# adam-kerrigan/pybader

Hardware: AMD Instinct MI355X
Metric: Mvoxels/s neargrid assign+refine on 512^3 grid (higher is better)
Workload: dtype f64; 1 GPU; 512^3 synthetic 8-Gaussian-atom cubic cell (BASELINE config 3), neargrid assign + neargrid edge refinement changed:2, density resident in HBM; method=neargrid, device_driven_slab_step=False, basins=8

## Files before the change

include/bader_hip.h:

```cpp
#ifndef BADER_HIP_H
#define BADER_HIP_H

#include <stdint.h>

#ifdef __cplusplus
extern "C" {
#endif

typedef struct xb_ctx xb_ctx;

enum { XB_OK = 0, XB_E_ARG = -1, XB_E_HIP = -2, XB_E_STATE = -3, XB_E_LIMIT = -4, XB_E_COMM = -5,
       XB_E_SHORT = -6  };

enum { XB_I8 = 1, XB_I16 = 2, XB_I32 = 4, XB_I64 = 8 };

enum { XB_METHOD_ONGRID = 0, XB_METHOD_NEARGRID = 1 };
enum { XB_REFINE_ALL = 0, XB_REFINE_CHANGED = 1 };

const char *xb_last_error(void);
int xb_device_count(void);
int xb_create(int device, xb_ctx **out);
void xb_destroy(xb_ctx *c);
int xb_sync(xb_ctx *c);
void *xb_stream(xb_ctx *c);
// ... 228 lines not shown
    XB_REGIONS_BOXES = 1,
    XB_REGIONS_BRICKS = 2
};
enum { XB_DROP_TABLE_AND_MAXIMA = 2 };
enum {
    XB_CHECK_NO_MIRROR = 1,
    XB_CHECK_GENERIC_WALKER = 2,
    XB_CHECK_FULL_TGRAD = 4,
    XB_CHECK_LIST_DILATE = 8,
    XB_CHECK_WIDE_HALO = 16,
    XB_CHECK_NO_EC_SHARE = 32,
    XB_CHECK_IO_GATHER = 64
};
#define XB_CHECK_BRICK_LOOKUP 128
#define XB_CHECK_VOXEL_SWEEP 256
#define XB_CHECK_GENERIC_RETRACE 512
enum {
    XB_DBG_EC_PASSES = 4,
    XB_DBG_SLAB_STATS = 16,
    XB_DBG_STAGE_WAIT = 32,
    XB_DBG_SHORT_TIERS = 64
};
#define XB_DBG_KEEP_RETRACE_OVERFLOW 128
int xb_set_option(xb_ctx *c, int key, int value);
int xb_host_alloc(int64_t bytes, void **out);
int xb_host_free(void *p);
int xb_memory_stats(xb_ctx *c, int64_t *bytes_total, int64_t *bytes_table, int64_t *bytes_scratch);
int xb_box_stats(xb_ctx *c, int64_t *n_boxes, int64_t *box_voxels);
int xb_brick_labels(xb_ctx *c, int32_t *out, int64_t capacity, int64_t dims[3]);
int xb_slow_path_stats(xb_ctx *c, int64_t *assign_total, int64_t *refine_total);
int xb_deferred_stats(xb_ctx *c, int64_t *refine_total);
int xb_sweep_stats(xb_ctx *c, int64_t *bit_sweeps, int64_t *voxel_sweeps);
int xb_retrace_stats(xb_ctx *c, int64_t *lean_launches, int64_t *generic_launches);
int xb_retrace_overflow(xb_ctx *c, int32_t *out, int64_t capacity, int64_t *n);
int xb_edge_list(xb_ctx *c, int32_t *out, int64_t capacity, int64_t *edges, int64_t *tiles_listed);
int xb_growth_stats(xb_ctx *c, int64_t *retries, int64_t *kill_launches);

int xb_comm_unique_id(uint8_t id_out[128]);
int xb_comm_init(xb_ctx *c, int rank, int nranks, const uint8_t id_in[128]);
int xb_comm_destroy(xb_ctx *c);
int xb_comm_exchange_planes(xb_ctx *c, int which, int n_send, const int32_t *send_peer, const int64_t *send_xa,
                            const int64_t *send_xb, int n_recv, const int32_t *recv_peer, const int64_t *recv_xa,
                            const int64_t *recv_xb);
int xb_comm_allreduce_i64(xb_ctx *c, int64_t *inout, int64_t n, int op);
int xb_comm_allgather_i64(xb_ctx *c, const int64_t *in, int64_t n, int64_t *out);
int xb_comm_share_brick_masks(xb_ctx *c, const int64_t *first, const int64_t *count);
int xb_comm_allgather_block(xb_ctx *c, int which, const int64_t *first, const int64_t *count);
int xb_comm_allreduce_block(xb_ctx *c);
int xb_comm_info(xb_ctx *c, int64_t out[4]);
int xb_comm_stats(xb_ctx *c, int64_t *bytes_sent);

#ifdef __cplusplus
}
#endif
#endif
```

pybader_amd/_lib.py:

```python
import ctypes as C
import threading
import os

import numpy as np

HERE = os.path.dirname(os.path.abspath(__file__))
LIB_PATH = os.environ.get('XB_LIBRARY') or os.path.join(HERE, 'libbader_hip.so')

METHODS = {'ongrid': 0, 'neargrid': 1}
REFINE_MODES = {'all': 0, 'changed': 1}
DTYPE_CODE = {np.dtype(np.int8): 1, np.dtype(np.int16): 2, np.dtype(np.int32): 4, np.dtype(np.int64): 8}
(XB_XC_EDGES, XB_XC_CHANGED, XB_XC_ESCAPED, XB_XC_TRAVELLING, XB_XC_SLOW, XB_XC_LOST, XB_XC_MINE, XB_XC_ROUNDS,
 XB_XC_COUNT) = range(9)
(XB_TIMER_ASSIGN, XB_TIMER_OG_MASKS, XB_TIMER_EDGE_FIND, XB_TIMER_REFINE_TRACE, XB_TIMER_MASKS_GROWTH, XB_TIMER_BRICK_MASKS,
 XB_TIMER_TRACE, XB_TIMER_BRICK_RECORDS, XB_TIMER_MOMENTS, XB_TIMER_ADJACENCY, XB_TIMER_MERGE, XB_TIMER_COUNT) = range(12)
XB_OPT_REGIONS = 1
XB_REGIONS_BOXES, XB_REGIONS_BRICKS = 1, 2
XB_OPT_CROSS_CHECK = 2
(XB_CHECK_NO_MIRROR, XB_CHECK_GENERIC_WALKER, XB_CHECK_FULL_TGRAD, XB_CHECK_LIST_DILATE, XB_CHECK_WIDE_HALO,
 XB_CHECK_NO_EC_SHARE, XB_CHECK_IO_GATHER) = (1, 2, 4, 8, 16, 32, 64)
CROSS_CHECK_BRICK_LOOKUP = 128
CROSS_CHECK_VOXEL_SWEEP = 256
CROSS_CHECK_GENERIC_RETRACE = 512
XB_OPT_DEBUG = 3
# ... 147 lines not shown
    'xb_isa_rho_bound': (_int, [_vp, _pdbl]),
    'xb_volume_assign': (_int, [_vp, _vp, _i64]),
    'xb_atom_assign': (_int, [_vp, _i64, _vp, _i64, _vp, _vp, _vp]),
    'xb_surface_distance': (_int, [_vp, _vp, _vp, _i64, _vp, _pi64]),
    'xb_volume_mask': (_int, [_vp, _i64, _vp]),
    'xb_label_sum': (_int, [_vp, _i64, _pdbl, _pi64]),
    'xb_set_table_window': (_int, [_vp, _i64]),
    'xb_table_build': (_int, [_vp, _pi64]),
    'xb_table_local_seeds': (_int, [_vp, _vp, _i64]),
    'xb_brick_masks': (_int, [_vp, C.POINTER(_vp), _pi64, _pi64, _pi64]),
    'xb_table_ties': (_int, [_vp, _pi64]),
    'xb_table_finish': (_int, [_vp, _vp, _i64, _i64]),
    'xb_labels_ptr': (_vp, [_vp]),
    'xb_known_ptr': (_vp, [_vp]),
    'xb_density_ptr': (_vp, [_vp]),
    'xb_plane_elems': (_i64, [_vp]),
    'xb_copy_planes': (_int, [_vp, _int, _int, _vp, _i64, _i64]),
    'xb_label_wire': (_int, [_vp, _int, _vp]),
    'xb_host_alloc': (_int, [_i64, _vp]),
    'xb_host_free': (_int, [_vp]),
    'xb_brick_masks_copy': (_int, [_vp, _int, _vp, _i64, _i64]),
    'xb_set_halo': (_int, [_vp, _i64]),
    'xb_kernel_time': (_int, [_vp, _int, _pdbl, _pi64]),
    'xb_kernel_time_reset': (_int, [_vp]),
    'xb_enable_timing': (_int, [_vp, _int]),
    'xb_set_option': (_int, [_vp, _int, _int]),
    'xb_box_stats': (_int, [_vp, _pi64, _pi64]),
    'xb_brick_labels': (_int, [_vp, _vp, _i64, _pi64]),
    'xb_slow_path_stats': (_int, [_vp, _pi64, _pi64]),
    'xb_deferred_stats': (_int, [_vp, _pi64]),
    'xb_sweep_stats': (_int, [_vp, _pi64, _pi64]),
    'xb_edge_list': (_int, [_vp, _vp, _i64, _pi64, _pi64]),
    'xb_retrace_stats': (_int, [_vp, _pi64, _pi64]),
    'xb_retrace_overflow': (_int, [_vp, _vp, _i64, _pi64]),
    'xb_growth_stats': (_int, [_vp, _pi64, _pi64]),
    'xb_comm_unique_id': (_int, [_vp]),
    'xb_comm_init': (_int, [_vp, _int, _int, _vp]),
    'xb_comm_destroy': (_int, [_vp]),
    'xb_comm_exchange_planes': (_int, [_vp, _int, _int, _vp, _pi64, _pi64, _int, _vp, _pi64, _pi64]),
    'xb_comm_allreduce_i64': (_int, [_vp, _pi64, C.c_int64, _int]),
    'xb_comm_allgather_i64': (_int, [_vp, _pi64, C.c_int64, _pi64]),
    'xb_comm_share_brick_masks': (_int, [_vp, _pi64, _pi64]),
    'xb_comm_allgather_block': (_int, [_vp, _int, _pi64, _pi64]),
    'xb_comm_allreduce_block': (_int, [_vp]),
    'xb_slab_supported': (_int, [_vp, _int, _pi64]),
    'xb_slab_assign_masks': (_int, [_vp, _int, _int]),
    'xb_slab_assign_trace': (_int, [_vp]),
    'xb_slab_assign_finish': (_int, [_vp, _pi64, _pi64]),
    'xb_slab_refine_pass': (_int, [_vp]),
    'xb_slab_walkers_round': (_int, [_vp, _int, _int]),
    'xb_slab_walk_layout': (_int, [_vp, _pi64]),
    'xb_slab_walk_send': (_int, [_vp, _i64]),
    'xb_slab_refine_counts': (_int, [_vp, _pi64, _pi64]),
    'xb_slab_block': (_int, [_vp, _int, C.POINTER(_vp), _pi64, _pi64, _pi64]),
    'xb_slab_block_copy': (_int, [_vp, _int, _int, _vp, _i64, _i64]),
    'xb_host_waits': (_int, [_pi64]),
    'xb_comm_stats': (_int, [_vp, _pi64]),
    'xb_comm_info': (_int, [_vp, _pi64]),
    'xb_memory_stats': (_int, [_vp, _pi64, _pi64, _pi64]),
}

_lib = None


class BaderHipError(RuntimeError):
    code = None
# ... 1045 lines not shown

    def brick_labels(self):
        dims = (C.c_int64 * 3)()
        check(self.lib.xb_brick_labels(self.h, None, 0, dims))
        out = np.zeros(tuple(int(d) for d in dims), np.int32)
        check(self.lib.xb_brick_labels(self.h, _ptr(out), out.size, dims))
        return out

    def slow_path_stats(self):
        a, b = C.c_int64(), C.c_int64()
        check(self.lib.xb_slow_path_stats(self.h, C.byref(a), C.byref(b)))
        return a.value, b.value

    def growth_stats(self):
        a, b = C.c_int64(), C.c_int64()
        check(self.lib.xb_growth_stats(self.h, C.byref(a), C.byref(b)))
        return a.value, b.value

    def deferred_stats(self):
        a = C.c_int64()
        check(self.lib.xb_deferred_stats(self.h, C.byref(a)))
        return a.value

    def sweep_stats(self):
        a, b = C.c_int64(), C.c_int64()
        check(self.lib.xb_sweep_stats(self.h, C.byref(a), C.byref(b)))
        return a.value, b.value

    def retrace_stats(self):
        a, b = C.c_int64(), C.c_int64()
        check(self.lib.xb_retrace_stats(self.h, C.byref(a), C.byref(b)))
        return a.value, b.value

    def retrace_overflow(self):
        n = C.c_int64()
        check(self.lib.xb_retrace_overflow(self.h, None, 0, C.byref(n)))
        out = np.zeros(n.value, np.int32)
        if n.value:
            check(self.lib.xb_retrace_overflow(self.h, _ptr(out), out.size, C.byref(n)))
        return out

    def edge_list(self):
        n, t = C.c_int64(), C.c_int64()
        check(self.lib.xb_edge_list(self.h, None, 0, C.byref(n), C.byref(t)))
        out = np.zeros(n.value, np.int32)
        if n.value:
            check(self.lib.xb_edge_list(self.h, _ptr(out), out.size, C.byref(n), C.byref(t)))
        return out, t.value

    def sync(self):
        check(self.lib.xb_sync(self.h))


def critical_lut():
    out = np.zeros(XB_CRITICAL_LUT_SIZE, np.uint8)
    check(load().xb_critical_lut(_ptr(out)))
    return out


def isosurface_table():
    out = np.zeros(XB_ISO_TABLE_SIZE, np.uint8)
    check(load().xb_isosurface_table(_ptr(out)))
    return out.reshape(6, 16, 8)


def hirshfeld_images(lattice, atoms_cart, species, r_cut):
# ... 40 lines not shown
```

pybader_amd/csrc/bader_hip.hip:

```cpp
#include "bader_kernels.h"
#include "../../include/bader_hip.h"
#include "ctx_state.h"
#include "ctx_buffers.h"

#include <algorithm>
#include <cmath>
#include <cstdarg>
#include <cstdio>
#include <cstring>
#include <locale.h>
#include <mutex>
#include <string>
#include <thread>
#include <vector>

static thread_local long long xb_waits = 0;
static inline hipError_t xb_counted_sync(hipStream_t s) { xb_waits++; return (hipStreamSynchronize)(s); }
#define hipStreamSynchronize(s) xb_counted_sync(s)

#include "k_common.h"
#include "k_masks.h"
#include "k_fused.h"
#include "k_trace.h"
#include "k_ongrid.h"
// ... 77 lines not shown
        int ec_qcap = EC_Q;
        int self_exchange = 0;
        int async_comm = 0;
        bool weight_no_labels = false;
    } opt;
    int *ec_share = nullptr;
    std::vector<int64_t> esc_starts, esc_offsets, esc_vox;
    unsigned long long *ec_pend = nullptr;
    int8_t *ec_pflag = nullptr;
    std::vector<int8_t> esc_complete;
    double vac_tol = 0.;
    bool regions_pending = false;
    bool buni_halo_safe = false;
    bool regions_neargrid = false;
    int n_walk = 0;
    int *walk = nullptr;
    int table_margin = -1;
    bool table_prebuilt = false;
    int table_stage = 0;
    std::vector<int> window_seeds;
    bool window_ties = true;
    bool slab_sparse = false;
    int ec_local_n = 0;
    int walk_n_out = 0;
    void *walk_out_dev = nullptr;
    std::vector<int64_t> walk_host, res_host;
    int walk_n_res = 0;
    void *walk_in = nullptr, *walk_out2 = nullptr, *walk_res = nullptr;
    long long walk_cap = 0;
    long long stat_deferred = 0;
    long long stat_bit_sweeps = 0, stat_voxel_sweeps = 0;
    long long stat_ovf_assign = 0, stat_ovf_refine = 0;
    long long stat_lean_retraces = 0, stat_generic_retraces = 0;
    std::vector<int> dbg_retrace_ovf;
    int *bres_last = nullptr;
    int *blab = nullptr;
    int nbk[3] = {0, 0, 0};
    bool brick_max_blanket = false;
    int grad_cover = 0;
    unsigned char *brick_rec = nullptr;
    unsigned long long *nb_tab = nullptr;
    void *xbuf = nullptr;
    int slab_rank = 0, slab_nranks = 0, slab_stage = 0;
    void *wbuf[2] = {nullptr, nullptr};
    void *wk_in = nullptr;
    int wbuf_ranks = 0, walk_last = -1, walk_round = 0, wcap = 0;
    int walk_send = 0;
    int grow_kill_launches = 6;
    long long stat_grow_retries = 0;
    bool defer_wait = false;
    bool pending_assign = false;
    int64_t pending_n_maxima = 0;
    int grad_rule = 0;
    int *labels = nullptr;
    int8_t *known = nullptr;
    int *first = nullptr;
    int *list = nullptr;
    int8_t *st = nullptr;
    void *stage = nullptr;
    size_t stage_bytes = 0;
    int *max_list = nullptr;
    int *max_aux = nullptr;
    int max_cap = 0;
    int *ovf_list = nullptr;
    int ovf_cap = 0;
    int *counters = nullptr;
// ... 204 lines not shown
    case XB_OPT_DROP_TABLE: if (value == XB_DROP_TABLE_AND_MAXIMA) drop_table_and_maxima(*c); else drop_table(*c); break;
    case XB_OPT_KILL_LAUNCHES: if ((ok = value >= 1)) c->grow_kill_launches = value; break;
    case XB_OPT_SELF_EXCHANGE: c->opt.self_exchange = value != 0; break;
    case XB_OPT_ASYNC_COMM: c->opt.async_comm = value != 0; break;
    case XB_OPT_WEIGHT_NO_LABELS: c->opt.weight_no_labels = value != 0; break;
    default: ok = false;
    }
    if (!ok) return fail(XB_E_ARG, "xb_set_option: unknown key %d", key);
    return XB_OK;
}
int xb_growth_stats(xb_ctx *c, int64_t *retries, int64_t *kill_launches) {
    if (!c) return fail(XB_E_ARG, "null ctx");
    if (retries) *retries = c->stat_grow_retries;
    if (kill_launches) *kill_launches = c->grow_kill_launches;
    return XB_OK;
}
int xb_deferred_stats(xb_ctx *c, int64_t *refine_total) {
    if (!c) return fail(XB_E_ARG, "null ctx");
    if (refine_total) *refine_total = c->stat_deferred;
    return XB_OK;
}
int xb_sweep_stats(xb_ctx *c, int64_t *bit_sweeps, int64_t *voxel_sweeps) {
    if (!c) return fail(XB_E_ARG, "null ctx");
    if (bit_sweeps) *bit_sweeps = c->stat_bit_sweeps;
    if (voxel_sweeps) *voxel_sweeps = c->stat_voxel_sweeps;
    return XB_OK;
}
int xb_retrace_stats(xb_ctx *c, int64_t *lean_launches, int64_t *generic_launches) {
    if (!c) return fail(XB_E_ARG, "null ctx");
    if (lean_launches) *lean_launches = c->stat_lean_retraces;
    if (generic_launches) *generic_launches = c->stat_generic_retraces;
    return XB_OK;
}
int xb_retrace_overflow(xb_ctx *c, int32_t *out, int64_t capacity, int64_t *n) {
    if (!c || !n || capacity < 0 || (capacity > 0 && !out)) return fail(XB_E_ARG, "xb_retrace_overflow: null ctx / count, or a capacity without a buffer");
    *n = (int64_t)c->dbg_retrace_ovf.size();
    if (capacity >= *n) {
        std::copy(c->dbg_retrace_ovf.begin(), c->dbg_retrace_ovf.end(), out);
        c->dbg_retrace_ovf.clear();
    }
    return XB_OK;
}
int xb_slow_path_stats(xb_ctx *c, int64_t *assign_total, int64_t *refine_total) {
    if (!c) return fail(XB_E_ARG, "null ctx");
    if (assign_total) *assign_total = c->stat_ovf_assign;
    if (refine_total) *refine_total = c->stat_ovf_refine;
    return XB_OK;
}
int xb_memory_stats(xb_ctx *c, int64_t *bytes_total, int64_t *bytes_table, int64_t *bytes_scratch) {
    if (!c || !c->has_grid) return fail(XB_E_STATE, "xb_memory_stats: no grid");
    const long long N = c->N;
    const long long table = c->grad_cap * (long long)sizeof(GradRec);
    const long long scratch = c->list_cap * 4 + (long long)c->stage_bytes + c->ec_buf_cap * 4 + (c->ec_pend ? 8 * N + 16 : 0) +
                              (long long)buf_counted_bytes(*c) ;
    const long long fixed = 8 * N  + 4 * N  + (N + 16)  + 4 * N  + N  +
                            2LL * c->max_cap * 4 + (long long)c->ovf_cap * 4 + c->blab_alloc * 13 + (long long)c->walk_cap * 3 * 80 +
                            (1 << 22) ;
    if (bytes_total) *bytes_total = fixed + table + scratch;
    if (bytes_table) *bytes_table = table;
    if (bytes_scratch) *bytes_scratch = scratch;
    return XB_OK;
}
int xb_box_stats(xb_ctx *c, int64_t *n_boxes, int64_t *box_voxels) {
    if (!c) return fail(XB_E_ARG, "null ctx");
    if (n_boxes) *n_boxes = c->n_boxes;
    if (box_voxels) *box_voxels = c->box_voxels;
// ... 76 lines not shown
```

pybader_amd/csrc/bader_kernels.h:

```cpp
#pragma once
#include <hip/hip_runtime.h>
#include <stdint.h>

struct Grid {
    int nx, ny, nz;
    int nyz;
    int x0, x1;
    int vx0, vlen;
    int wx0, wlen;
    int wbase, ntot;
    int main_ties;
    double T[9];
    double dist[27];
};

struct GridS {
    int nx, ny, nz, nyz;
    int x0, x1, vx0, vlen;
    int wx0, wlen;
    int wbase, ntot;
    int main_ties;
    double T[9];
    double dsym[14];
};
// ... 113 lines not shown
#define XB_KEY_BITS 21
#define XB_NB_SHIFT 11
constexpr __host__ __device__ int nb_side(int pos) { return pos < 4 ? -1 : 1; }
constexpr __host__ __device__ int nb_index(int cx, int cy, int cz) { return cx + 2 * cy + 4 * cz - 1; }
constexpr __host__ __device__ int key_low(int code, int og, int nb) { return code | (og << 6) | ((nb & 127) << XB_NB_SHIFT); }
constexpr __host__ __device__ int low_code(int bits) { return bits & 63; }
constexpr __host__ __device__ int low_og(int bits) { return (bits >> 6) & 31; }
constexpr __host__ __device__ bool low_nb_norec(int bits, int cx, int cy, int cz) {
    return (cx | cy | cz) != 0 && ((bits >> (XB_NB_SHIFT + nb_index(cx, cy, cz))) & 1) != 0;
}
namespace nb_check {
constexpr bool subsets_ok() {
    for (int m = 1; m < 8; m++) {
        const int cx = m & 1, cy = (m >> 1) & 1, cz = m >> 2;
        if (nb_index(cx, cy, cz) != m - 1) return false;
        for (int code = 0; code < 64; code += 21)
            for (int og = 0; og < 27; og += 13) {
                const int one = key_low(code, og, 1 << (m - 1)), rest = key_low(code, og, 127 & ~(1 << (m - 1)));
                if (low_code(one) != code || low_og(one) != og || low_code(rest) != code || low_og(rest) != og) return false;
                if (one >> XB_KEY_BITS || rest >> XB_KEY_BITS) return false;
                for (int k = 1; k < 8; k++) {
                    if (low_nb_norec(one, k & 1, (k >> 1) & 1, k >> 2) != (k == m)) return false;
                    if (low_nb_norec(rest, k & 1, (k >> 1) & 1, k >> 2) != (k != m)) return false;
                }
                if (low_nb_norec(one, 0, 0, 0) || low_nb_norec(key_low(code, og, 127), 0, 0, 0)) return false;
            }
    }
    return true;
}
static_assert(subsets_ok(), "7 neighbour bits, one per subset of crossed axes, clear of the step code and the ongrid successor");
static_assert(nb_side(0) == -1 && nb_side(1) == -1 && nb_side(3) == -1 && nb_side(4) == 1 && nb_side(6) == 1 && nb_side(7) == 1,
              "the low side is within reach from positions 0-1 only, the high side from 6-7 only");
static_assert(key_low(XB_STAY_CODE, 26, 127) == 0x3FEBF && key_low(63, 31, 127) < (1 << 18), "bits 18-20 stay 0");
}
__device__ __forceinline__ double pack_key(double rho, int code, int og, int nb = 0) {
    return __longlong_as_double((__double_as_longlong(rho) & ~0x1FFFFFLL) | (long long)key_low(code, og, nb));
}
__device__ __forceinline__ double key_floor(double rho) {
    const long long b = __double_as_longlong(rho);
    return __longlong_as_double(b >= 0 ? (b & ~0x1FFFFFLL) : (b | 0x1FFFFFLL));
}
__device__ __forceinline__ int key_bits(double key) { return (int)(__double_as_longlong(key) & 0x1FFFFFLL); }
__device__ __forceinline__ int key_code(double key) { return low_code(key_bits(key)); }
__device__ __forceinline__ int key_og(double key) { return low_og(key_bits(key)); }
static_assert((1 << XB_KEY_BITS) - 1 == 0x1FFFFF, "key_bits / key_floor / pack_key share one mask");

__device__ __forceinline__ int wrap_u(int q, int n) {
    unsigned u = min((unsigned)q, (unsigned)(q + n));
    return (int)min(u, u - (unsigned)n);
}
__device__ __forceinline__ int lin3f(const GridL &g, int x, int y, int z) {
    if (g.use24) return (int)__umul24(__umul24(x, g.ny) + y, g.nz) + z;
    return (x * g.ny + y) * g.nz + z;
}
__device__ __forceinline__ void ng_move_t(const GridL &g, int px, int py, int pz, const GradRec &rec, int code,
                                          double &dr0, double &dr1, double &dr2, int &qx, int &qy, int &qz) {
    int id;
    dr0 += rec.r0; id = rha_cs(dr0); qx = px + ((code & 3) - 1) + id; dr0 -= (double)id;
    dr1 += rec.r1; id = rha_cs(dr1); qy = py + (((code >> 2) & 3) - 1) + id; dr1 -= (double)id;
    dr2 += rec.r2; id = rha_cs(dr2); qz = pz + ((code >> 4) - 1) + id; dr2 -= (double)id;
    qx = wrap_u(qx, g.nx); qy = wrap_u(qy, g.ny); qz = wrap_u(qz, g.nz);
}

template <typename GT>
__device__ __forceinline__ void og_step(const double *__restrict__ rho, const GT &g, const double *__restrict__ dist,
                                        int px, int py, int pz, double ctr, int &qx, int &qy, int &qz) {
// ... 89 lines not shown
```

pybader_amd/csrc/host_stages.h:

```cpp

enum { BB_TOTAL = 1 << 20, BB_REGMAX = 1 << 16, BB_REGFIRST = 1 << 17 };

static bool table_windowed(const xb_ctx *c) { return c->g.wlen < c->g.nx; }
static int small_grid(const Grid &g) { return g.nx < 16 || g.ny < 16 || g.nz < 80; }
static int trace_maxsteps(const Grid &g) { return 8 * (g.nx + g.ny + g.nz) + 64; }
static const int *slab_regions_of(const xb_ctx *c) {
    const Grid &g = c->g;
    return (table_windowed(c) && c->blab && c->regions_labels && !c->has_vacuum && (c->grad_rule == 2 || c->slab_sparse) &&
            g.nx % 8 == 0 && g.ny % 8 == 0 && g.nz % 8 == 0) ? c->blab : nullptr;
}

static_assert(CT_REDO == CT_N_MAX + 15, "a host-driven assignment zeroes CT_N_MAX .. CT_REDO at once");
static int begin_assignment(xb_ctx *c, int *counts, int n, bool invalidate) {
    HIPCHK(hipMemsetAsync(counts, 0, n * sizeof(int), c->stream));
    if (!c->first_clean) {
        k_fill<int><<<4096, TPB, 0, c->stream>>>(c->first, XB_INT_MAX, c->N);
        HIPCHK(hipGetLastError());
    }
    c->first_clean = false;
    c->regions_pending = false;
    if (invalidate) { drop_label_marks(*c); drop_edge_lists(*c); }
    return XB_OK;
}

// ... 37 lines not shown
    const int nbr = nb0 * nb1 * nb2;
    int *fs = c->fs;
    k_seed_bricks<<<(nbr + 255) / 256, 256, 0, c->stream>>>(nbr, bmask, bmaxv, fs, seed, buf0, box_max, box_first);
    if (chase) {
        k_grow_parent<<<(nbr + TPB - 1) / TPB, TPB, 0, c->stream>>>(nb0, nb1, nb2, bmask, bpot, seed, buf1);
        k_grow_chase<<<(nbr + TPB - 1) / TPB, TPB, 0, c->stream>>>(nbr, buf1, seed, buf0, 4 * (nb0 + nb1 + nb2) + 64, fs);
    } else
        k_seed_finish<<<1, 1, 0, c->stream>>>(fs);
    const int long_schedule = 2 * ((std::max(std::max(nb0, nb1), nb2) + BG - 1) / BG) + 12;
    const int launches = chase ? std::min(long_schedule, c->grow_kill_launches) : long_schedule;
    const dim3 ggrid((nb2 + BG - 1) / BG, (nb1 + BG - 1) / BG, (nb0 + BG - 1) / BG);
    for (int l = 0; l < launches; l++)
        k_brick_grow_dev<<<ggrid, BG * BG * BG, 0, c->stream>>>(nb0, nb1, nb2, bmask, seed, buf0, buf1, fs, BG, 0);
    k_grow_finish<<<64, TPB, 0, c->stream>>>(nbr, seed, buf0, buf1, fs, c->blab_buf, box_first, bmask, c->brick_rec, 0, chase && launches < long_schedule ? 1 : 0);
}

static void launch_window_bricks(xb_ctx *c, int *list, int *count, const int *skip) {
    const Grid &g = c->g;
    const int nb0 = c->nbk[0], per_plane = c->nbk[1] * c->nbk[2], nbr = nb0 * per_plane;
    const int w0 = g.wx0 / BRK, wn = g.wlen / BRK, run1 = std::min(wn, nb0 - w0);
    const unsigned grid = (nbr + 16 * TPB - 1) / (16 * TPB);
    k_brick_walk_list<<<grid, TPB, 0, c->stream>>>(nbr, w0 * per_plane, (w0 + run1) * per_plane, c->blab, list, count, skip);
    if (wn > run1) k_brick_walk_list<<<grid, TPB, 0, c->stream>>>(nbr, 0, (wn - run1) * per_plane, c->blab, list, count, skip);
}

static bool launch_persistent_trace(xb_ctx *c, bool lean_ok, bool part, const int *box_max, const int *walk, int has_vacuum, int *bres) {
    const Grid &g = c->g;
    const int groups = std::max(1, c->trace_waves / XB_TRACE_WAVES);
    const int lean = lean_ok && light(g).use24 && c->opt.lean ? ((long long)g.wlen * g.nyz <= (1LL << 27) ? 4 : 3) : 0;
    const bool window = table_windowed(c);
    int *ovf = window ? (int *)c->stage : c->ovf_list;
    const int ovf_cap = window ? (int)std::min<size_t>(c->stage_bytes / sizeof(int), 0x7fffffffu) : c->ovf_cap;
    const bool nb = lean && !window && !part && nb_bits_ok(c);
    auto kernel = !lean ? k_ng_trace_g<2, 0>
                : nb ? (lean == 4 ? k_ng_trace_g<2, 4, false, false, true> : k_ng_trace_g<2, 3, false, false, true>)
                : window ? (lean == 4 ? k_ng_trace_g<2, 4, true> : k_ng_trace_g<2, 3, true>)
                : part ? (lean == 4 ? k_ng_trace_g<2, 4, false, true> : k_ng_trace_g<2, 3, false, true>)
                : (lean == 4 ? k_ng_trace_g<2, 4> : k_ng_trace_g<2, 3>);
    kernel<<<groups, XB_WAVE * XB_TRACE_WAVES, 0, c->stream>>>(light(g), c->grad, box_max, c->blab, c->nbk[1], c->nbk[2], walk, c->fs, c->labels,
                                                               c->first, c->max_list, c->max_cap, ovf, ovf_cap, trace_maxsteps(g), has_vacuum,
                                                               8, 1, lean ? bres : nullptr);
    if (window)
        k_ng_trace_list<2><<<512, TPB, 0, c->stream>>>(light(g), c->grad, box_max, c->blab, c->nbk[1], c->nbk[2], ovf, c->fs + FS_N_OVF, c->labels,
                                                       c->first, c->max_list, c->fs + FS_N_MAX, c->max_cap, c->ovf_list, c->counters + CT_N_OVF,
                                                       c->ovf_cap, trace_maxsteps(g), c->rho, c->dist_dev, has_vacuum);
    return lean != 0;
}

enum { BUNI_NONE, BUNI_SCAN, BUNI_MIXED };
static void launch_relabel(xb_ctx *c, int *fs, int n_maxima, bool regions, const int *box_max, int buni, const int *bres) {
    const Grid &g = c->g;
    const GridL gl = light(g);
    const int nb1 = c->nbk[1], nb2 = c->nbk[2], nbr = c->nbk[0] * nb1 * nb2;
    const int *gate = fs ? fs + FS_SORT_OK : nullptr, *n_walk_dev = fs ? fs + FS_N_WALK : nullptr;
    int *ubuf = reinterpret_cast<int *>(c->st);
    if (regions) {
        const int v = g.nz % 4 == 0 ? 4 : 1;
        (v == 4 ? k_relabel_regions_brick<4> : k_relabel_regions_brick<1>)<<<dim3((g.nz / v + 63) / 64, nb1, (g.x1 - g.x0 + 3) / 4), TPB, 0, c->stream>>>(
            gl, c->labels, c->first, c->blab, nb1, nb2, box_max, fs, gate, fs ? -1 : c->n_boxes);
        if (buni == BUNI_MIXED) k_fill<int><<<(nbr + 4 * TPB - 1) / (4 * TPB), TPB, 0, c->stream>>>(ubuf, XB_MIXED, nbr);
        if (buni != BUNI_NONE && bres)
            k_buni_after_relabel<<<(nbr + 255) / 256, 256, 0, c->stream>>>(nbr, c->blab, box_max, c->first, ubuf, gate, c->walk, n_walk_dev, bres);
        else if (buni != BUNI_NONE) {
            k_buni_after_relabel<<<(nbr + 255) / 256, 256, 0, c->stream>>>(nbr, c->blab, box_max, c->first, ubuf, gate, nullptr, nullptr, nullptr);
            if (fs) k_label_uniform_list<<<2048, TPB, 0, c->stream>>>(gl, c->labels, nb1, nb2, c->walk, 0, n_walk_dev, gate, ubuf);
            else if (c->n_walk)
// ... 53 lines not shown
```

pybader_amd/csrc/k_trace.h:

```cpp
#pragma once

__global__ __launch_bounds__(TPB) void k_fill_certain(GridL g, const int *__restrict__ blab, int nb1, int nb2,
                                                      const int *__restrict__ box_max, int *labels, int *first,
                                                      int *max_list, int *max_count, int max_cap, const int *skip = nullptr) {
    if (skip && *skip) return;
    const int vbeg = g.x0 * g.nyz, vend = g.x1 * g.nyz;
    const int v = vbeg + blockIdx.x * TPB + threadIdx.x;
    const bool in = v < vend;
    int result = -1;
    bool has = false;
    if (in) {
        const int x = v / g.nyz;
        const int r = v - x * g.nyz;
        const int y = r / g.nz, z = r - y * g.nz;
        const int b = blab[((x >> 3) * nb1 + (y >> 3)) * nb2 + (z >> 3)];
        if (b > 0 && labels[v] != -1) {
            result = box_max[b - 1];
            if (result != v && labels[result] == -1) result = -1;
            labels[v] = result;
            has = result >= 0;
        }
    }
    note_maximum_wave(has, result, in ? v : 0, first, max_list, max_count, max_cap);
}
// ... 185 lines not shown
                    result = -2;
                    moving = false;
                } else {
                    w.push(lq, nr.key);
                    px = qx; py = qy; pz = qz; lp = lq; rec = nr;
                }
            }
        }
    }
    if (has_vacuum && valid && result >= 0 && result != v && labels[result] == -1) result = -1;
    if (valid) labels[v] = result;
    note_maximum_wave(valid && result >= 0, result, v, first, max_list, max_count, max_cap);
    if (valid && result == -2) {
        const int k = atomicAdd(ovf_count, 1);
        if (k < ovf_cap) ovf_list[k] = v;
    }
}
__device__ __forceinline__ int wrap3(int q, int n) {
    return (int)min(min((unsigned)q, (unsigned)(q + n)), (unsigned)(q - n));
}
__device__ __forceinline__ int mad24(int a, int b, int c) {
    int r;
    asm("v_mad_u32_u24 %0, %1, %2, %3" : "=v"(r) : "v"(a), "s"(b), "v"(c));
    return r;
}
__device__ __forceinline__ int lin24(const GridL &g, int x, int y, int z) { return mad24(mad24(x, g.ny, y), g.nz, z); }
template <bool OFF32>
__device__ __forceinline__ GradRec fetch_rec_o(const GradRec *__restrict__ G, int l) {
    if (OFF32) return *reinterpret_cast<const GradRec *>(reinterpret_cast<const char *>(G) + ((unsigned)l << 5));
    return fetch_rec(G, l);
}
constexpr int XB_TRACE_WAVES = 4;
__shared__ GradRec xb_s_rec[512];
template <bool OFF32, bool CACHE, bool WINDOW = false, bool NB = false>
__device__ __forceinline__ int ng_walk_lean(const GridL &g, const GradRec *__restrict__ G, const int *__restrict__ box_max,
                                             const int *__restrict__ blab, int nb1, int nb2, int sx, int sy, int sz,
                                             int *labels, int *first, int *max_list, int *max_count, int max_cap,
                                             int *ovf_list, int *ovf_count, int ovf_cap, int maxsteps, bool has_vacuum) {
    static_assert(!NB || (CACHE && !WINDOW), "neighbour bits: the whole-grid table of the group trace");
    const int v = lin24(g, sx, sy, sz);
    const int lab0 = has_vacuum ? labels[v] : 0;
    const int ox8 = sx & ~7, oy8 = sy & ~7, oz8 = sz & ~7;
    GradRec rec = CACHE ? xb_s_rec[((sx & 7) << 6) | ((sy & 7) << 3) | (sz & 7)] : fetch_rec_o<OFF32>(G, WINDOW ? rec_slot(g, v) : v);
    int result = -1;
    int px = sx, py = sy, pz = sz, steps = 0;
    double dr0 = 0., dr1 = 0., dr2 = 0.;
    int i0 = v, i1 = -1;
    bool norec = false;
    double k0 = rec.key, k1 = -1.7976931348623157e308, m_old = -1.7976931348623157e308;
#ifdef XB_DEBUG_COUNT
    int dbg_lane_steps = 0;
#endif
    if (lab0 != -1) for (;;) {
        const int bits = key_bits(rec.key);
        const double t0 = dr0 + rec.r0, t1 = dr1 + rec.r1, t2 = dr2 + rec.r2;
        const int id0 = rha_cs(t0), id1 = rha_cs(t1), id2 = rha_cs(t2);
        const int m0 = (bits & 3) + id0 - 1, m1 = ((bits >> 2) & 3) + id1 - 1, m2 = ((bits >> 4) & 3) + id2 - 1;
        int cross = NB ? (((px ^ (px + m0)) >> 3) != 0) | ((((py ^ (py + m1)) >> 3) != 0) << 1) | ((((pz ^ (pz + m2)) >> 3) != 0) << 2) : 0;
        px += m0; py += m1; pz += m2;
        dr0 = t0 - (double)id0; dr1 = t1 - (double)id1; dr2 = t2 - (double)id2;
        if (__builtin_amdgcn_ballot_w64((unsigned)px >= (unsigned)g.nx || (unsigned)py >= (unsigned)g.ny || (unsigned)pz >= (unsigned)g.nz) != 0) {
            px = wrap3(px, g.nx); py = wrap3(py, g.ny); pz = wrap3(pz, g.nz);
        }
        int lq = lin24(g, px, py, pz);
        const bool og_move = (bits & 63) == XB_STAY_CODE || lq == i0 || lq == i1;
        bool at_max = false;
        if (__builtin_amdgcn_ballot_w64(og_move) != 0) {
            if (og_move) {
                const int og = (bits >> 6) & 31;
                int ox, oy, oz;
                og_offsets(og, ox, oy, oz);
                at_max = og == XB_OG_SELF;
                dr0 = dr1 = dr2 = 0.;
                const int ux = wrap3(px - m0, g.nx), uy = wrap3(py - m1, g.ny), uz = wrap3(pz - m2, g.nz);
                if (NB) cross = (((ux ^ (ux + ox)) >> 3) != 0) | ((((uy ^ (uy + oy)) >> 3) != 0) << 1) | ((((uz ^ (uz + oz)) >> 3) != 0) << 2);
                px = wrap3(ux + ox, g.nx);
                py = wrap3(uy + oy, g.ny);
                pz = wrap3(uz + oz, g.nz);
                lq = lin24(g, px, py, pz);
            }
        }
        int bl = 0;
        const bool own = CACHE && (unsigned)((px ^ ox8) | (py ^ oy8) | (pz ^ oz8)) < 8u;
        const bool in_win = !WINDOW || own || plane_in_window(g, px);
        if (NB) norec = cross != 0 && ((bits >> (XB_NB_SHIFT - 1) >> cross) & 1) != 0;
        if (own) rec = xb_s_rec[((px & 7) << 6) | ((py & 7) << 3) | (pz & 7)];
        else if (NB) {
            if (!norec) rec = fetch_rec_o<OFF32>(G, lq);
        } else {
            rec = fetch_rec_o<OFF32>(G, WINDOW ? (in_win ? rec_slot(g, lq) : 0) : lq);
            const unsigned bidx = (unsigned)mad24(mad24(px >> 3, nb1, py >> 3), nb2, pz >> 3);
            bl = *reinterpret_cast<const int *>(reinterpret_cast<const char *>(blab) + (bidx << 2));
        }
        steps++;
#ifdef XB_DEBUG_COUNT
        dbg_lane_steps++;
#endif
        if (NB && norec) break;
        const bool arrived = bl > 0 && !at_max;
        const bool undecided = (!og_move && rec.key <= m_old) || steps > maxsteps || (WINDOW && !in_win) || bl == XB_NOREC;
        if (arrived) result = box_max[bl - 1];
        else if (at_max) result = i0;
        else if (undecided) result = -2;
        if (arrived || at_max || undecided) break;
        m_old = max_raw(m_old, k1);
        i1 = i0; k1 = k0;
        i0 = lq; k0 = rec.key;
    }
    if (NB && norec) {
        const unsigned bidx = (unsigned)mad24(mad24(px >> 3, nb1, py >> 3), nb2, pz >> 3);
        const int bl = *reinterpret_cast<const int *>(reinterpret_cast<const char *>(blab) + (bidx << 2));
        result = bl > 0 ? box_max[bl - 1] : -2;
    }
#ifdef XB_DEBUG_COUNT
    if (xb_dbg_steps) xb_dbg_steps[v] = (signed char)min(dbg_lane_steps, 127);
#endif
    if (has_vacuum && result >= 0 && result != v && labels[result] == -1) result = -1;
    labels[v] = result;
    note_maximum_wave(result >= 0, result, v, first, max_list, max_count, max_cap);
    if (result == -2) {
        const int k = atomicAdd(ovf_count, 1);
        if (k < ovf_cap) ovf_list[k] = v;
    }
    return result;
}
__device__ __forceinline__ void brick_sub_voxel(int b, int sub, int lane, int nb1, int nb2, int &sx, int &sy, int &sz) {
    const int b0 = b / (nb1 * nb2), b1 = (b / nb2) % nb1, b2 = b % nb2;
    sx = b0 * 8 + ((sub >> 2) << 2) + (lane >> 4);
    sy = b1 * 8 + ((sub & 3) << 1) + ((lane >> 3) & 1);
    sz = b2 * 8 + (lane & 7);
}
template <int K, bool WIN>
__global__ __launch_bounds__(TPB) void k_ng_trace(GridL g, const GradRec *__restrict__ G,
                                                  const int *__restrict__ box_max, const int *__restrict__ blab,
                                                  int nb1, int nb2, const int *__restrict__ walk, int n_walk,
                                                  int *labels, int *first,
                                                  int *max_list, int *max_count, int max_cap, int *ovf_list,
                                                  int *ovf_count, int ovf_cap, int maxsteps, int opt,
                                                  const double *__restrict__ rho, const double *__restrict__ gc, int has_vacuum) {
    int blk = blockIdx.x;
    if (opt & 2) {
        const int per = gridDim.x >> 3;
        if (blk < (per << 3)) blk = (blk & 7) * per + (blk >> 3);
    }
    const int wpb = blockDim.x / XB_WAVE;
    const int wave = blk * wpb + threadIdx.x / XB_WAVE;
// ... 105 lines not shown
            if (CACHE) {
                constexpr int PER = 512 / (XB_WAVE * XB_TRACE_WAVES);
                const int b = walk[base >> 3];
                prev_brick = b;
                const int b0 = b / (nb1 * nb2), b1 = (b / nb2) % nb1, b2 = b % nb2;
                GradRec tmp[PER];
#pragma unroll
                for (int k = 0; k < PER; k++) {
                    const int t = threadIdx.x + k * XB_WAVE * XB_TRACE_WAVES;
                    int cx = b0 * 8 + (t >> 6), cy = b1 * 8 + ((t >> 3) & 7), cz = b2 * 8 + (t & 7);
                    if (PART) { cx = min(cx, g.nx - 1); cy = min(cy, g.ny - 1); cz = min(cz, g.nz - 1); }
                    const int lt = lin24(g, cx, cy, cz);
                    tmp[k] = fetch_rec(G, WINDOW ? rec_slot(g, lt) : lt);
                }
#pragma unroll
                for (int k = 0; k < PER; k++) xb_s_rec[threadIdx.x + k * XB_WAVE * XB_TRACE_WAVES] = tmp[k];
                __syncthreads();
            }
#ifdef XB_DEBUG_COUNT
            pr_load += clock64() - pr_b;
#endif
            for (;;) {
                int i = 0;
                if (lane == 0) i = atomicAdd(&s_next, 1);
                const int item = base + __builtin_amdgcn_readfirstlane(i);
                if (item >= stop) break;
                int sx, sy, sz;
                brick_sub_voxel(walk[item >> 3], item & 7, lane, nb1, nb2, sx, sy, sz);
                if (PART) { sx = min(sx, g.nx - 1); sy = min(sy, g.ny - 1); sz = min(sz, g.nz - 1); }
                if (LEAN) {
#ifdef XB_DEBUG_COUNT
                    const long long pr_c = clock64();
#endif
                    const int res = ng_walk_lean<LEAN == 4, CACHE, WINDOW, NB>(g, G, box_max, blab, nb1, nb2, sx, sy, sz, labels, first, max_list, &fs[FS_N_MAX],
                                                                max_cap, ovf_list, &fs[FS_N_OVF], ovf_cap, maxsteps, has_vacuum != 0);
#ifdef XB_DEBUG_COUNT
                    pr_walk += clock64() - pr_c;
#endif
                    if (CACHE && bres) {
                        volatile int *w = s_w;
                        if (lane == 0) w[item - base] = res;
                        if (w[item - base] != res) *(volatile int *)&s_mixed = 1;
                    }
                }
                else
                    ng_walk_wave<K, false>(g, G, box_max, blab, nb1, nb2, true, sx, sy, sz, labels, first, max_list, &fs[FS_N_MAX],
                                           max_cap, ovf_list, &fs[FS_N_OVF], ovf_cap, maxsteps, nullptr, nullptr, has_vacuum != 0);
            }
        }
    }
#ifdef XB_DEBUG_COUNT
    if (lane == 0 && blockIdx.x < 2048) {
        unsigned long long *o = xb_dbg + 64 + 6 * (blockIdx.x * XB_TRACE_WAVES + (threadIdx.x >> 6));
        o[0] = (unsigned long long)pr_walk; o[1] = (unsigned long long)(clock64() - pr_t0); o[2] = (unsigned long long)pr_wait;
        o[3] = (unsigned long long)pr_load; o[4] = pr_e0; o[5] = (unsigned long long)wall_clock64();
        if (threadIdx.x == 0) xb_dbg[64 + 6 * 8192 + blockIdx.x] = (unsigned long long)pr_bricks;
    }
#endif
    if (CACHE && bres) {
        __syncthreads();
        if (threadIdx.x == 0) verdict();
    }
}

__global__ __launch_bounds__(TPB) void k_list_unfinished(GridL g, const int *__restrict__ walk, const int *n_walk, int nb1, int nb2,
                                                         const int *__restrict__ labels, int *out, int *out_count, int out_cap) {
    __shared__ int s_buf[BlockAppender<2>::CAP], s_n[2];
    BlockAppender<2> app;
// ... 107 lines not shown
```

Baseline: 45240 Mvoxels/s.

## Walk neargrid traces with a packed 10-bit-per-axis position in a sliding window

Adds a specialised walker for the neighbour-bits trace path. It keeps the voxel position as a single packed unsigned (three 10-bit fields relative to a 512-wide window), and the step delta, brick-ownership test, LDS slot, brick-crossing index and bounds check each become a few integer ops on that word. Per-axis wrap logic and the extra bookkeeping move into a rare rebase function. This aims to cut ALU and register cost per step in the hot trace loop, at the price of intricate bit tricks guarded by constexpr self-checks. Trace-launch counters and a stats API are also added.

```diff
diff --git a/include/bader_hip.h b/include/bader_hip.h
--- a/include/bader_hip.h
+++ b/include/bader_hip.h
@@ -284,6 +284,7 @@
 int xb_deferred_stats(xb_ctx *c, int64_t *refine_total);
 int xb_sweep_stats(xb_ctx *c, int64_t *bit_sweeps, int64_t *voxel_sweeps);
 int xb_retrace_stats(xb_ctx *c, int64_t *lean_launches, int64_t *generic_launches);
+int xb_trace_stats(xb_ctx *c, int64_t *nb_lean_launches, int64_t *lookup_lean_launches, int64_t *generic_launches);
 int xb_retrace_overflow(xb_ctx *c, int32_t *out, int64_t capacity, int64_t *n);
 int xb_edge_list(xb_ctx *c, int32_t *out, int64_t capacity, int64_t *edges, int64_t *tiles_listed);
 int xb_growth_stats(xb_ctx *c, int64_t *retries, int64_t *kill_launches);
diff --git a/pybader_amd/_lib.py b/pybader_amd/_lib.py
--- a/pybader_amd/_lib.py
+++ b/pybader_amd/_lib.py
@@ -203,6 +203,7 @@
     'xb_sweep_stats': (_int, [_vp, _pi64, _pi64]),
     'xb_edge_list': (_int, [_vp, _vp, _i64, _pi64, _pi64]),
     'xb_retrace_stats': (_int, [_vp, _pi64, _pi64]),
+    'xb_trace_stats': (_int, [_vp, _pi64, _pi64, _pi64]),
     'xb_retrace_overflow': (_int, [_vp, _vp, _i64, _pi64]),
     'xb_growth_stats': (_int, [_vp, _pi64, _pi64]),
     'xb_comm_unique_id': (_int, [_vp]),
@@ -1314,6 +1315,11 @@
         check(self.lib.xb_retrace_stats(self.h, C.byref(a), C.byref(b)))
         return a.value, b.value
 
+    def trace_stats(self):
+        a, b, g = C.c_int64(), C.c_int64(), C.c_int64()
+        check(self.lib.xb_trace_stats(self.h, C.byref(a), C.byref(b), C.byref(g)))
+        return a.value, b.value, g.value
+
     def retrace_overflow(self):
         n = C.c_int64()
         check(self.lib.xb_retrace_overflow(self.h, None, 0, C.byref(n)))
diff --git a/pybader_amd/csrc/bader_hip.hip b/pybader_amd/csrc/bader_hip.hip
--- a/pybader_amd/csrc/bader_hip.hip
+++ b/pybader_amd/csrc/bader_hip.hip
@@ -133,6 +133,7 @@
     long long stat_bit_sweeps = 0, stat_voxel_sweeps = 0;
     long long stat_ovf_assign = 0, stat_ovf_refine = 0;
     long long stat_lean_retraces = 0, stat_generic_retraces = 0;
+    long long stat_nb_traces = 0, stat_lookup_traces = 0, stat_generic_traces = 0;
     std::vector<int> dbg_retrace_ovf;
     int *bres_last = nullptr;
     int *blab = nullptr;
@@ -403,6 +404,13 @@
     if (generic_launches) *generic_launches = c->stat_generic_retraces;
     return XB_OK;
 }
+int xb_trace_stats(xb_ctx *c, int64_t *nb_lean_launches, int64_t *lookup_lean_launches, int64_t *generic_launches) {
+    if (!c) return fail(XB_E_ARG, "null ctx");
+    if (nb_lean_launches) *nb_lean_launches = c->stat_nb_traces;
+    if (lookup_lean_launches) *lookup_lean_launches = c->stat_lookup_traces;
+    if (generic_launches) *generic_launches = c->stat_generic_traces;
+    return XB_OK;
+}
 int xb_retrace_overflow(xb_ctx *c, int32_t *out, int64_t capacity, int64_t *n) {
     if (!c || !n || capacity < 0 || (capacity > 0 && !out)) return fail(XB_E_ARG, "xb_retrace_overflow: null ctx / count, or a capacity without a buffer");
     *n = (int64_t)c->dbg_retrace_ovf.size();
diff --git a/pybader_amd/csrc/bader_kernels.h b/pybader_amd/csrc/bader_kernels.h
--- a/pybader_amd/csrc/bader_kernels.h
+++ b/pybader_amd/csrc/bader_kernels.h
@@ -169,6 +169,92 @@
 static_assert(nb_side(0) == -1 && nb_side(1) == -1 && nb_side(3) == -1 && nb_side(4) == 1 && nb_side(6) == 1 && nb_side(7) == 1,
               "the low side is within reach from positions 0-1 only, the high side from 6-7 only");
 static_assert(key_low(XB_STAY_CODE, 26, 127) == 0x3FEBF && key_low(63, 31, 127) < (1 << 18), "bits 18-20 stay 0");
+}
+
+constexpr unsigned PW_ONES = 1u | (1u << 10) | (1u << 20);
+constexpr unsigned PW_LOW3 = 7u * PW_ONES, PW_EIGHTS = 8u * PW_ONES, PW_GUARD = 512u * PW_ONES;
+constexpr unsigned PW_NO_MOVE = 0x40000000u;
+constexpr unsigned PW_NO_BRICK = 0xFFFFFFFFu;
+constexpr int PW_SPAN = 512;
+constexpr __host__ __device__ unsigned pw_pack(int fx, int fy, int fz) { return ((unsigned)fx << 20) + ((unsigned)fy << 10) + (unsigned)fz; }
+constexpr __host__ __device__ int pw_x(unsigned p) { return (int)(p >> 20); }
+constexpr __host__ __device__ int pw_y(unsigned p) { return (int)((p >> 10) & 1023u); }
+constexpr __host__ __device__ int pw_z(unsigned p) { return (int)(p & 1023u); }
+constexpr __host__ __device__ int pw_win(int a, int n) {
+    const int w = (a & ~7) - PW_SPAN / 2, top = n > PW_SPAN ? n - PW_SPAN : 0;
+    return w < 0 ? 0 : (w > top ? top : w);
+}
+constexpr __host__ __device__ unsigned pw_hiw(int nx, int ny, int nz) {
+    return pw_pack(nx < PW_SPAN ? PW_SPAN - nx : 0, ny < PW_SPAN ? PW_SPAN - ny : 0, nz < PW_SPAN ? PW_SPAN - nz : 0);
+}
+constexpr __host__ __device__ bool pw_left(unsigned p, unsigned hiw) { return ((p | (p + hiw)) & PW_GUARD) != 0; }
+constexpr __host__ __device__ unsigned pw_delta(int bits, int id0, int id1, int id2) {
+    const unsigned code = (unsigned)bits & 63u;
+    return (((code * 0x100100u) & 0x300C00u) | (code >> 4)) + pw_pack(id0, id1, id2) - PW_ONES;
+}
+constexpr __host__ __device__ int pw_sext10(unsigned d) { return (int)((d + 512u) & 1023u) - 512; }
+constexpr __host__ __device__ int pw_delta_z(unsigned d) { return pw_sext10(d); }
+constexpr __host__ __device__ int pw_delta_y(unsigned d) { return pw_sext10((d - (unsigned)pw_delta_z(d)) >> 10); }
+constexpr __host__ __device__ int pw_delta_x(unsigned d) { return pw_sext10((((d - (unsigned)pw_delta_z(d)) >> 10) - (unsigned)pw_delta_y(d)) >> 10); }
+constexpr __host__ __device__ bool pw_own(unsigned p, unsigned own_high) { return (p & ~PW_LOW3) == own_high; }
+constexpr __host__ __device__ int pw_slot(unsigned p) { return (int)((((p & PW_LOW3) * 0x4081u) >> 14) & 511u); }
+constexpr __host__ __device__ int pw_cross(unsigned p, unsigned d) {
+    const unsigned s = ((p & PW_LOW3) | PW_EIGHTS) + d;
+    return (int)((((~s & PW_EIGHTS) * 0x400801u) >> 23) & 7u);
+}
+namespace pw_check {
+constexpr bool row_ok(int lx, int ly) {
+    const int org[3][3] = {{0, 256, 504}, {504, 0, 256}, {8, 496, 0}};
+    for (int lz = 0; lz < 8; lz++)
+        for (int k = 0; k < 3; k++) {
+            const int ox = org[k][0], oy = org[k][1], oz = org[k][2];
+            const unsigned p = pw_pack(ox + lx, oy + ly, oz + lz), high = pw_pack(ox, oy, oz);
+            if (pw_x(p) != ox + lx || pw_y(p) != oy + ly || pw_z(p) != oz + lz) return false;
+            if (!pw_own(p, high) || pw_slot(p) != ((lx << 6) | (ly << 3) | lz) || pw_left(p, 0)) return false;
+            for (int m0 = -2; m0 <= 2; m0++)
+                for (int m1 = -2; m1 <= 2; m1++)
+                    for (int m2 = -2; m2 <= 2; m2++) {
+                        const unsigned d = pw_pack(m0, m1, m2), q = p + d;
+                        if (pw_delta_x(d) != m0 || pw_delta_y(d) != m1 || pw_delta_z(d) != m2) return false;
+                        const int qx = ox + lx + m0, qy = oy + ly + m1, qz = oz + lz + m2;
+                        const bool cx = (lx + m0) < 0 || (lx + m0) > 7, cy = (ly + m1) < 0 || (ly + m1) > 7, cz = (lz + m2) < 0 || (lz + m2) > 7;
+                        if (pw_cross(p, d) != (cx ? 1 : 0) + (cy ? 2 : 0) + (cz ? 4 : 0)) return false;
+                        if ((cx || cy || cz) && pw_cross(p, d) != nb_index(cx, cy, cz) + 1) return false;
+                        const bool out = qx < 0 || qx >= PW_SPAN || qy < 0 || qy >= PW_SPAN || qz < 0 || qz >= PW_SPAN;
+                        if (pw_left(q, 0) != out) return false;
+                        if (!out && (pw_x(q) != qx || pw_y(q) != qy || pw_z(q) != qz || pw_own(q, high) != !(cx || cy || cz))) return false;
+                        if ((d == 0) != (m0 == 0 && m1 == 0 && m2 == 0)) return false;
+                    }
+        }
+    return true;
+}
+constexpr bool codes_ok() {
+    for (int code = 0; code < 64; code++)
+        for (int id = 0; id < 27; id++) {
+            const int id0 = id / 9 - 1, id1 = (id / 3) % 3 - 1, id2 = id % 3 - 1;
+            const int m0 = (code & 3) + id0 - 1, m1 = ((code >> 2) & 3) + id1 - 1, m2 = ((code >> 4) & 3) + id2 - 1;
+            const unsigned d = pw_delta(code | (21 << 6) | (127 << XB_NB_SHIFT), id0, id1, id2);
+            if (d != pw_pack(m0, m1, m2)) return false;
+            if (d + pw_pack(-m0, -m1, -m2) != 0 || d + PW_NO_MOVE == 0) return false;
+            for (int e = 0; e < 27; e++)
+                if ((d + pw_pack(e / 9 - 1, (e / 3) % 3 - 1, e % 3 - 1) == 0) != (m0 == 1 - e / 9 && m1 == 1 - (e / 3) % 3 && m2 == 1 - e % 3)) return false;
+        }
+    for (int n = 8; n <= 1032; n += 8) {
+        const unsigned hiw = pw_hiw(n, 4096, n);
+        for (int o = 0; o < n; o += 8) {
+            const int w = pw_win(o, n);
+            if (w < 0 || (w & 7) || o - w < 0 || o - w + 8 > PW_SPAN || (n >= PW_SPAN && w + PW_SPAN > n) || (n < PW_SPAN && w != 0)) return false;
+        }
+        const int w = pw_win(n - 8, n);
+        for (int a = n - 3; a < n + 3; a++)
+            if (pw_left(pw_pack(a - w, 5, a - w), hiw) != (a >= n)) return false;
+        if (!pw_left(pw_pack(-1, 5, 5), hiw) || !pw_left(pw_pack(5, -2, 5), hiw) || !pw_left(pw_pack(5, 5, -3), hiw)) return false;
+    }
+    return true;
+}
+template <int K> struct rows { static_assert(row_ok(K >> 3, K & 7), "packed position: own test, LDS slot, crossing index, window test"); rows<K - 1> rest; };
+template <> struct rows<-1> {};
+static_assert(sizeof(rows<63>) > 0 && codes_ok(), "packed position: pack / unpack and the move equal the per-axis formulas");
 }
 __device__ __forceinline__ double pack_key(double rho, int code, int og, int nb = 0) {
     return __longlong_as_double((__double_as_longlong(rho) & ~0x1FFFFFLL) | (long long)key_low(code, og, nb));
diff --git a/pybader_amd/csrc/host_stages.h b/pybader_amd/csrc/host_stages.h
--- a/pybader_amd/csrc/host_stages.h
+++ b/pybader_amd/csrc/host_stages.h
@@ -93,6 +93,7 @@
     int *ovf = window ? (int *)c->stage : c->ovf_list;
     const int ovf_cap = window ? (int)std::min<size_t>(c->stage_bytes / sizeof(int), 0x7fffffffu) : c->ovf_cap;
     const bool nb = lean && !window && !part && nb_bits_ok(c);
+    (nb ? c->stat_nb_traces : lean ? c->stat_lookup_traces : c->stat_generic_traces)++;
     auto kernel = !lean ? k_ng_trace_g<2, 0>
                 : nb ? (lean == 4 ? k_ng_trace_g<2, 4, false, false, true> : k_ng_trace_g<2, 3, false, false, true>)
                 : window ? (lean == 4 ? k_ng_trace_g<2, 4, true> : k_ng_trace_g<2, 3, true>)
diff --git a/pybader_amd/csrc/k_trace.h b/pybader_amd/csrc/k_trace.h
--- a/pybader_amd/csrc/k_trace.h
+++ b/pybader_amd/csrc/k_trace.h
@@ -241,12 +241,11 @@
 }
 constexpr int XB_TRACE_WAVES = 4;
 __shared__ GradRec xb_s_rec[512];
-template <bool OFF32, bool CACHE, bool WINDOW = false, bool NB = false>
+template <bool OFF32, bool CACHE, bool WINDOW = false>
 __device__ __forceinline__ int ng_walk_lean(const GridL &g, const GradRec *__restrict__ G, const int *__restrict__ box_max,
                                              const int *__restrict__ blab, int nb1, int nb2, int sx, int sy, int sz,
                                              int *labels, int *first, int *max_list, int *max_count, int max_cap,
                                              int *ovf_list, int *ovf_count, int ovf_cap, int maxsteps, bool has_vacuum) {
-    static_assert(!NB || (CACHE && !WINDOW), "neighbour bits: the whole-grid table of the group trace");
     const int v = lin24(g, sx, sy, sz);
     const int lab0 = has_vacuum ? labels[v] : 0;
     const int ox8 = sx & ~7, oy8 = sy & ~7, oz8 = sz & ~7;
@@ -255,7 +254,6 @@
     int px = sx, py = sy, pz = sz, steps = 0;
     double dr0 = 0., dr1 = 0., dr2 = 0.;
     int i0 = v, i1 = -1;
-    bool norec = false;
     double k0 = rec.key, k1 = -1.7976931348623157e308, m_old = -1.7976931348623157e308;
 #ifdef XB_DEBUG_COUNT
     int dbg_lane_steps = 0;
@@ -265,7 +263,6 @@
         const double t0 = dr0 + rec.r0, t1 = dr1 + rec.r1, t2 = dr2 + rec.r2;
         const int id0 = rha_cs(t0), id1 = rha_cs(t1), id2 = rha_cs(t2);
         const int m0 = (bits & 3) + id0 - 1, m1 = ((bits >> 2) & 3) + id1 - 1, m2 = ((bits >> 4) & 3) + id2 - 1;
-        int cross = NB ? (((px ^ (px + m0)) >> 3) != 0) | ((((py ^ (py + m1)) >> 3) != 0) << 1) | ((((pz ^ (pz + m2)) >> 3) != 0) << 2) : 0;
         px += m0; py += m1; pz += m2;
         dr0 = t0 - (double)id0; dr1 = t1 - (double)id1; dr2 = t2 - (double)id2;
         if (__builtin_amdgcn_ballot_w64((unsigned)px >= (unsigned)g.nx || (unsigned)py >= (unsigned)g.ny || (unsigned)pz >= (unsigned)g.nz) != 0) {
@@ -282,7 +279,6 @@
                 at_max = og == XB_OG_SELF;
                 dr0 = dr1 = dr2 = 0.;
                 const int ux = wrap3(px - m0, g.nx), uy = wrap3(py - m1, g.ny), uz = wrap3(pz - m2, g.nz);
-                if (NB) cross = (((ux ^ (ux + ox)) >> 3) != 0) | ((((uy ^ (uy + oy)) >> 3) != 0) << 1) | ((((uz ^ (uz + oz)) >> 3) != 0) << 2);
                 px = wrap3(ux + ox, g.nx);
                 py = wrap3(uy + oy, g.ny);
                 pz = wrap3(uz + oz, g.nz);
@@ -292,11 +288,8 @@
         int bl = 0;
         const bool own = CACHE && (unsigned)((px ^ ox8) | (py ^ oy8) | (pz ^ oz8)) < 8u;
         const bool in_win = !WINDOW || own || plane_in_window(g, px);
-        if (NB) norec = cross != 0 && ((bits >> (XB_NB_SHIFT - 1) >> cross) & 1) != 0;
         if (own) rec = xb_s_rec[((px & 7) << 6) | ((py & 7) << 3) | (pz & 7)];
-        else if (NB) {
-            if (!norec) rec = fetch_rec_o<OFF32>(G, lq);
-        } else {
+        else {
             rec = fetch_rec_o<OFF32>(G, WINDOW ? (in_win ? rec_slot(g, lq) : 0) : lq);
             const unsigned bidx = (unsigned)mad24(mad24(px >> 3, nb1, py >> 3), nb2, pz >> 3);
             bl = *reinterpret_cast<const int *>(reinterpret_cast<const char *>(blab) + (bidx << 2));
@@ -305,7 +298,6 @@
 #ifdef XB_DEBUG_COUNT
         dbg_lane_steps++;
 #endif
-        if (NB && norec) break;
         const bool arrived = bl > 0 && !at_max;
         const bool undecided = (!og_move && rec.key <= m_old) || steps > maxsteps || (WINDOW && !in_win) || bl == XB_NOREC;
         if (arrived) result = box_max[bl - 1];
@@ -316,11 +308,96 @@
         i1 = i0; k1 = k0;
         i0 = lq; k0 = rec.key;
     }
-    if (NB && norec) {
-        const unsigned bidx = (unsigned)mad24(mad24(px >> 3, nb1, py >> 3), nb2, pz >> 3);
+#ifdef XB_DEBUG_COUNT
+    if (xb_dbg_steps) xb_dbg_steps[v] = (signed char)min(dbg_lane_steps, 127);
+#endif
+    if (has_vacuum && result >= 0 && result != v && labels[result] == -1) result = -1;
+    labels[v] = result;
+    note_maximum_wave(result >= 0, result, v, first, max_list, max_count, max_cap);
+    if (result == -2) {
+        const int k = atomicAdd(ovf_count, 1);
+        if (k < ovf_cap) ovf_list[k] = v;
+    }
+    return result;
+}
+__device__ __forceinline__ int pw_lin(const GridL &g, unsigned p, int lb) { return mad24(mad24(pw_x(p), g.ny, pw_y(p)), g.nz, pw_z(p)) + lb; }
+__device__ __forceinline__ void pw_rebase(const GridL &g, int nb1, int nb2, int bx8, int by8, int bz8, unsigned p_old, unsigned d,
+                                          unsigned &p, unsigned &own_high, int &lb, int &wb) {
+    const int wx = (wb / (nb1 * nb2)) << 3, wy = ((wb / nb2) % nb1) << 3, wz = (wb % nb2) << 3;
+    const int ax = wrap3(wx + pw_x(p_old) + pw_delta_x(d), g.nx), ay = wrap3(wy + pw_y(p_old) + pw_delta_y(d), g.ny),
+              az = wrap3(wz + pw_z(p_old) + pw_delta_z(d), g.nz);
+    const int ux = pw_win(ax, g.nx), uy = pw_win(ay, g.ny), uz = pw_win(az, g.nz);
+    p = pw_pack(ax - ux, ay - uy, az - uz);
+    lb = lin24(g, ux, uy, uz);
+    wb = ((ux >> 3) * nb1 + (uy >> 3)) * nb2 + (uz >> 3);
+    const int rx = bx8 - ux, ry = by8 - uy, rz = bz8 - uz;
+    own_high = (unsigned)(rx | ry | rz) < (unsigned)PW_SPAN ? pw_pack(rx, ry, rz) : PW_NO_BRICK;
+}
+template <bool OFF32>
+__device__ __forceinline__ int ng_walk_packed(const GridL &g, const GradRec *__restrict__ G, const int *__restrict__ box_max,
+                                               const int *__restrict__ blab, int nb1, int nb2, int bx8, int by8, int bz8, int sx, int sy, int sz,
+                                               int *labels, int *first, int *max_list, int *max_count, int max_cap,
+                                               int *ovf_list, int *ovf_count, int ovf_cap, int maxsteps, bool has_vacuum) {
+    const int v = lin24(g, sx, sy, sz);
+    const int lab0 = has_vacuum ? labels[v] : 0;
+    GradRec rec = xb_s_rec[((sx & 7) << 6) | ((sy & 7) << 3) | (sz & 7)];
+    const unsigned hiw = pw_hiw(g.nx, g.ny, g.nz);
+    int lb, wb;
+    unsigned p, own_high;
+    {
+        const int wx = pw_win(bx8, g.nx), wy = pw_win(by8, g.ny), wz = pw_win(bz8, g.nz);
+        p = pw_pack(sx - wx, sy - wy, sz - wz);
+        own_high = pw_pack(bx8 - wx, by8 - wy, bz8 - wz);
+        lb = lin24(g, wx, wy, wz);
+        wb = ((wx >> 3) * nb1 + (wy >> 3)) * nb2 + (wz >> 3);
+    }
+    int steps = 0;
+    double dr0 = 0., dr1 = 0., dr2 = 0.;
+    unsigned d_prev = PW_NO_MOVE;
+    double k0 = rec.key, k1 = -1.7976931348623157e308, m_old = -1.7976931348623157e308;
+    unsigned d = PW_NO_MOVE;
+    int norec = 0;
+#ifdef XB_DEBUG_COUNT
+    int dbg_lane_steps = 0;
+#endif
+    if (lab0 != -1) for (;;) {
+        const int bits = key_bits(rec.key);
+        const double t0 = dr0 + rec.r0, t1 = dr1 + rec.r1, t2 = dr2 + rec.r2;
+        const int id0 = rha_cs(t0), id1 = rha_cs(t1), id2 = rha_cs(t2);
+        d = pw_delta(bits, id0, id1, id2);
+        dr0 = t0 - (double)id0; dr1 = t1 - (double)id1; dr2 = t2 - (double)id2;
+        const bool og_move = min(min(((unsigned)bits & 63u) ^ (unsigned)XB_STAY_CODE, d), d + d_prev) == 0u;
+        if (og_move) {
+            int ox, oy, oz;
+            og_offsets((bits >> 6) & 31, ox, oy, oz);
+            dr0 = dr1 = dr2 = 0.;
+            d = pw_pack(ox, oy, oz);
+        }
+        const int cross = pw_cross(p, d);
+        const unsigned p_old = p;
+        p += d;
+        if (pw_left(p, hiw)) pw_rebase(g, nb1, nb2, bx8, by8, bz8, p_old, d, p, own_high, lb, wb);
+        const bool own = pw_own(p, own_high);
+        norec = (((bits >> XB_NB_SHIFT) << 1) >> cross) & 1;
+        if (own) rec = xb_s_rec[pw_slot(p)];
+        else if (!norec) rec = fetch_rec_o<OFF32>(G, pw_lin(g, p, lb));
+        steps++;
+#ifdef XB_DEBUG_COUNT
+        dbg_lane_steps++;
+#endif
+        if (norec != 0 || d == 0u || (!og_move && rec.key <= m_old) || steps > maxsteps) break;
+        m_old = max_raw(m_old, k1);
+        k1 = k0; k0 = rec.key;
+        d_prev = d;
+    }
+    asm volatile("" : "+v"(norec), "+v"(d));
+    int result = -1;
+    if (norec != 0) {
+        const unsigned bidx = (unsigned)(mad24(mad24(pw_x(p) >> 3, nb1, pw_y(p) >> 3), nb2, pw_z(p) >> 3) + wb);
         const int bl = *reinterpret_cast<const int *>(reinterpret_cast<const char *>(blab) + (bidx << 2));
         result = bl > 0 ? box_max[bl - 1] : -2;
-    }
+    } else if (d == 0u) result = pw_lin(g, p, lb);
+    else if (lab0 != -1) result = -2;
 #ifdef XB_DEBUG_COUNT
     if (xb_dbg_steps) xb_dbg_steps[v] = (signed char)min(dbg_lane_steps, 127);
 #endif
@@ -492,8 +569,14 @@
 #ifdef XB_DEBUG_COUNT
                     const long long pr_c = clock64();
 #endif
-                    const int res = ng_walk_lean<LEAN == 4, CACHE, WINDOW, NB>(g, G, box_max, blab, nb1, nb2, sx, sy, sz, labels, first, max_list, &fs[FS_N_MAX],
-                                                                max_cap, ovf_list, &fs[FS_N_OVF], ovf_cap, maxsteps, has_vacuum != 0);
+                    int res;
+                    if constexpr (NB) {
+                        const int wbrick = walk[item >> 3];
+                        res = ng_walk_packed<LEAN == 4>(g, G, box_max, blab, nb1, nb2, (wbrick / (nb1 * nb2)) << 3, ((wbrick / nb2) % nb1) << 3, (wbrick % nb2) << 3,
+                                                        sx, sy, sz, labels, first, max_list, &fs[FS_N_MAX], max_cap, ovf_list, &fs[FS_N_OVF], ovf_cap, maxsteps, has_vacuum != 0);
+                    } else
+                        res = ng_walk_lean<LEAN == 4, CACHE, WINDOW>(g, G, box_max, blab, nb1, nb2, sx, sy, sz, labels, first, max_list, &fs[FS_N_MAX],
+                                                                     max_cap, ovf_list, &fs[FS_N_OVF], ovf_cap, maxsteps, has_vacuum != 0);
 #ifdef XB_DEBUG_COUNT
                     pr_walk += clock64() - pr_c;
 #endif
```

New measurement: 45930 Mvoxels/s (median of 6 runs). +1.5%, better.
